# lambdaclass/simpleworks

Measured on AMD Instinct MI355X. Metric: Marlin prove() constraints/sec at 2^20 R1CS; G1 MSM points/sec, higher is better.
Workload: dtype u32 limbs (384-bit Montgomery Fq for G1, 256-bit Fr); 1 GPU; marlin_prove: synthetic R1CS, 2^20 constraints = variables = non-zeros per matrix (|H| = |K| = 2^20), SRS + proving key device resident; per_gpu_units=1048576, multi_gpu=replicas (one proof per rank)

## Files before the change

### simpleworks_amd/_lib.py

```python
import ctypes
import json
import os

import numpy as np

_HERE = os.path.dirname(os.path.abspath(__file__))
LIB_PATH = os.environ.get("SWM_LIB_PATH") or os.path.join(_HERE, "libswmarlin.so")

_u64p = ctypes.POINTER(ctypes.c_uint64)
_u32p = ctypes.POINTER(ctypes.c_uint32)
_vp = ctypes.c_void_p
_sz = ctypes.c_size_t
_int = ctypes.c_int

ABI = {
    "swm_version": (_int, []),
    "swm_strerror": (ctypes.c_char_p, [_int]),
    "swm_init": (_int, [_int, ctypes.POINTER(_vp)]),
    "swm_destroy": (None, [_vp]),
    "swm_last_error": (ctypes.c_char_p, [_vp]),
    "swm_set_stream": (_int, [_vp, _vp]),
    "swm_set_msm_sharding": (_int, [_vp, ctypes.c_uint, ctypes.c_uint, _vp, _vp]),
    "swm_rccl_unique_id": (_int, [ctypes.c_void_p]),
    "swm_rccl_init": (_int, [_vp, ctypes.c_void_p, ctypes.c_uint, ctypes.c_uint]),
# ... 466 lines not shown

    def selftest_ntt_cosets(self, coeffs_mont, log_n, ks):
        src = np.ascontiguousarray(coeffs_mont, dtype=np.uint64).reshape(-1, 4).copy()
        kk = np.ascontiguousarray(ks, dtype=np.uint64).reshape(-1)
        out = np.zeros((kk.size << log_n, 4), dtype=np.uint64)
        self._check(self.lib.swm_selftest_poly(self.h, 9, src.ctypes.data, src.shape[0], log_n, _p64(np.zeros(4, np.uint64)),
                                               _p64(kk), kk.size, out.ctypes.data), "swm_selftest_poly")
        return out.reshape(kk.size, 1 << log_n, 4)

    def selftest_intt_cosets3(self, evals_mont, log_n):
        ev = np.ascontiguousarray(evals_mont, dtype=np.uint64).reshape(-1, 4).copy()
        out = np.zeros_like(ev)
        self._poly(10, ev, ev.shape[0], log_n, None, None, out)
        return out

    def selftest_scan(self, words):
        w = np.ascontiguousarray(words, dtype=np.uint32).reshape(-1)
        out = np.zeros(w.size + 1, dtype=np.uint32)
        self._poly(8, w, w.size, 0, None, None, out)
        return out[:-1], int(out[-1])

    def selftest_sample_fr(self, rng, need):
        out = np.zeros((max(need, 1), 4), dtype=np.uint64)
        self._check(self.lib.swm_selftest_sample_fr(self.h, rng.h, need, _p64(out)), "swm_selftest_sample_fr")
        return out[:need]

    def selftest_mul_throughput(self, which, threads, iters):
        ms = ctypes.c_float(0)
        self._check(self.lib.swm_selftest_mul_throughput(self.h, which, threads, iters, ctypes.byref(ms)),
                    "swm_selftest_mul_throughput")
# ... 2 lines not shown
```

### simpleworks_amd/csrc/devops.cuh

```cuda
#pragma once
#include <chrono>
#include <exception>
#include <functional>
#include <utility>
#include <atomic>
#include "context.h"
#include "ff.cuh"
#include "fill.cuh"
#include "fr29.cuh"
#include "host/chacha.h"
#include "host/marlin_types.h"

namespace swm {

int ntt_run(swm_ctx* ctx, void* d_data, unsigned log_n, int inverse, int coset);
int ntt_run_from(swm_ctx* ctx, void* d_data, unsigned log_n, int inverse, int coset, const void* first_src, size_t src_len);
int ntt_cosets_fwd(swm_ctx* ctx, const void* coeffs, size_t len, unsigned log_n, const unsigned* ks, unsigned ncos, void* out);
int ntt_cosets_inv(swm_ctx* ctx, void* data, unsigned log_n, unsigned ncos);
int ntt_sharded_run(swm_ctx* ctx, void* d_local, unsigned log_n, int inverse, int blocks_in);
struct SpmvPlanHost {
    uint64_t nnz = 0, max_row = 0;
    std::vector<uint32_t> chunks, lrows;
};
struct SpmvPlan {
    uint64_t nnz = 0, max_row = 0;
    const uint32_t* d_chunks = nullptr;
    const uint32_t* d_lrows = nullptr;
    uint32_t n_chunks = 0, n_lrows = 0;
};
void spmv_plan_build(const uint32_t* rowptr, size_t rows, SpmvPlanHost* plan);
int spmv_run(swm_ctx* ctx, const void* d_rowptr, const void* d_col, const void* d_val, const void* d_z, void* d_out,
             size_t rows, const SpmvPlan* plan = nullptr);
int batch_inverse_run(swm_ctx* ctx, void* d, size_t n);
// ... 847 lines not shown
```

### simpleworks_amd/csrc/marlin.hip

```cpp
#include <stdlib.h>
#include <string.h>
#include <algorithm>
#include <chrono>
#include <functional>
#include <memory>
#include "devops.cuh"
#include "g1.cuh"
#include "host/ahp.h"

#include "msm.h"
using namespace swm;

#define LAUNCHX(ctx, name, kernel, grid, block, shmem, ...)                         \
    do {                                                                            \
        prof_begin(ctx, name);                                                      \
        hipLaunchKernelGGL(kernel, grid, block, shmem, (ctx)->stream, __VA_ARGS__); \
        prof_end(ctx);                                                              \
        hip_check(ctx, hipGetLastError(), name);                                    \
    } while (0)

#include "host/pk_codec.h"
#include "host/host_handles.h"
struct swm_srs {
    ~swm_srs() {
// ... 972 lines not shown
}
#ifndef SWM_OUTER_COSETS
#define SWM_OUTER_COSETS 1
#endif
static constexpr uint64_t OUTER_COSETS_MIN_H = 16;
struct Cosets3 {
    Fr p0, p1, p2;
};
__device__ __forceinline__ Cosets3 cosets3_solve(const Fr& u0, const Fr& u1, const Fr& u2, const Fr& iota, const Fr& half) {
    const Fr p1 = fp_mul(fp_sub(u0, u2), half);
    const Fr e = fp_mul(fp_add(u0, u2), half);
    const Fr d = fp_sub(u1, fp_mul(iota, p1));
    return {fp_mul(fp_add(e, d), half), p1, fp_mul(fp_sub(e, d), half)};
}
static Fr fr_half() { return fp_inv(fp_from_u64<Fr>(2)); }
struct RAlphaNumerators {
    Fr n0, n1, n2, n3;
};
RAlphaNumerators r_alpha_numerators(const Fr& alpha, unsigned logH, uint64_t M) {
    Fr aH = alpha;
    for (unsigned i = 0; i < logH; i++) aH = fp_sqr(aH);
    Fr i4 = HDomain(M).gen;
    for (unsigned i = 0; i < logH; i++) i4 = fp_sqr(i4);
    return {fp_sub(aH, fp_one<Fr>()), fp_sub(aH, i4), fp_sub(aH, fp_sqr(i4)), fp_sub(aH, fp_mul(fp_sqr(i4), i4))};
}
struct IndexOnB {
    const Fr *ar, *ac, *arc, *av;
    const Fr *br, *bc, *brc, *bv;
    const Fr *cr, *cc, *crc, *cv;
};
// ... 388 lines not shown
        hip_check(ctx, hipMemcpyAsync(s.e_ra.p + H, e12.p, 2 * H * sizeof(Fr), hipMemcpyDeviceToDevice, ctx->stream), "copy");
    }
    {
        DVec e_t = on_cosets12(ctx, s, s.t_poly.p, H);
        Fr* out = s.q1.p + H;
        const Fr *pra = s.e_ra.p + H, *pza = s.e_za.p, *pzb = s.e_zb.p, *pt = e_t.p, *pz = s.e_z.p;
        ew(ctx, "round2_pointwise", 2 * H, [=] __device__(size_t i) {
            Fr a = pza[i], b = pzb[i];
            Fr summed = fp_add(fp_add(fp_mul(eta_c, fp_mul(a, b)), fp_mul(eta_a, a)), fp_mul(eta_b, b));
            out[i] = fp_sub(fp_mul(pra[i], summed), fp_mul(pz[i], pt[i]));
        });
        s.e_za.release();
        s.e_zb.release();
        s.e_z.release();
    }
    rc_check(ctx, ntt_cosets_inv(ctx, s.q1.p, pk.logH, 3));
    s.h1 = DVec(ctx, 3 * H);
    s.g1x = DVec(ctx, H);
    const Fr* q = s.q1.p;
    const Fr* mp = s.mask.p;
    Fr *h = s.h1.p, *g = s.g1x.p;
    const Fr iota = HDomain(4).gen, half = fr_half();
    ew(ctx, "q1_cosets_solve_div_vh", H, [=] __device__(size_t j) {
        const Cosets3 c = cosets3_solve(q[j], q[j + H], q[j + 2 * H], iota, half);
        const Fr p0 = fp_add(c.p0, mp[j]), p1 = fp_add(c.p1, mp[j + H]), p2 = fp_add(c.p2, mp[j + 2 * H]);
        const Fr hj = fp_add(p1, p2);
        h[j] = hj;
        h[j + H] = p2;
        h[j + 2 * H] = fp_zero<Fr>();
        g[j] = fp_add(p0, hj);
    });
// ... 69 lines not shown
                        {&s.P_t.rand, &s.P_g1.rand, &s.P_h1.rand}, s.comms2.data());
    if (unsat && !ctx->emulated_exchange)
        throw MarlinError(SWM_ERR_UNSATISFIED, "outer sumcheck does not hold: constraint system is not satisfied");
}

void round3_polys(swm_ctx* ctx, const swm_pk& pk, ProveState& s) {
    const uint64_t K = s.K, Bsz = s.Bsz;
    const Fr alpha = s.st.alpha, beta = s.st.beta;
    const Fr eta_a = s.st.eta_a, eta_b = s.st.eta_b, eta_c = s.st.eta_c;
    const Fr vhab = fp_mul(s.dh.vanishing(alpha), s.dh.vanishing(beta));
    s.f = DVec(ctx, K);
    const bool f_cosets = SWM_OUTER_COSETS && !s.sp.r3 && Bsz == 4 * K && K >= OUTER_COSETS_MIN_H;
    DVec f_K;
    {
        DVec inv(ctx, 3 * K);
        for (int m = 0; m < 3; m++) {
            Fr* out = inv.p + (size_t)m * K;
            const Fr *rk = pk.ar[m].row_K.p, *ck = pk.ar[m].col_K.p;
            ew(ctx, "round3_den_K", K, [=] __device__(size_t i) { out[i] = fp_mul(fp_sub(beta, rk[i]), fp_sub(alpha, ck[i])); });
        }
        rc_check(ctx, batch_inverse_run(ctx, inv.p, 3 * K));
        Fr* out = s.f.p;
        const Fr *ia = inv.p, *ib = inv.p + K, *ic = inv.p + 2 * K;
        const Fr *va = pk.ar[0].val_K.p, *vb = pk.ar[1].val_K.p, *vc = pk.ar[2].val_K.p;
        if (f_cosets) {
            f_K = DVec(ctx, K);
            out = f_K.p;
        }
        ew(ctx, "round3_f_K", K, [=] __device__(size_t i) {
            Fr t = fp_add(fp_add(fp_mul(fp_mul(eta_a, va[i]), ia[i]), fp_mul(fp_mul(eta_b, vb[i]), ib[i])),
                          fp_mul(fp_mul(eta_c, vc[i]), ic[i]));
            out[i] = fp_mul(vhab, t);
        });
        if (f_cosets) rc_check(ctx, ntt_run_from(ctx, s.f.p, pk.logK, 1, 0, f_K.p, K));
        else dv_ntt(ctx, s.f, pk.logK, true);
// ... 7 lines not shown
    const Round3Challenges ch{alpha, beta, fp_mul(beta, alpha), eta_a, eta_b, eta_c, vhab};
    if (s.sp.r3) {
        const size_t Bloc = Bsz / s.sp.SG, Bblk = Bloc / s.sp.SG, Kl = K / s.sp.SG, s_rank = s.sp.rank;
        DVec e_f = shard_evals(ctx, s.sp, s.f.p, K, pk.logB);
        DVec ab(ctx, Bloc);
        Fr* out = ab.p;
        const Fr* pf = e_f.p;
        ew(ctx, "round3_pointwise_B", Bloc, [=] __device__(size_t p) {
            const size_t i = Bloc * (p / Bblk) + s_rank * Bblk + (p % Bblk);
            out[p] = round3_a_minus_bf(ix, ch, i, pf[p]);
        });
        rc_check(ctx, ntt_sharded_run(ctx, ab.p, pk.logB, 1, 1));
        DVec loc(ctx, 3 * Kl);
        div_vk(ctx, ab.p, Kl, Bloc, loc.p);
        shard_gather_cyclic(ctx, loc.p, 3 * Kl, s.sp.slog_g, s.h2.p, 3 * K);
    } else if (f_cosets) {
        static const unsigned ks[3] = {1, 2, 3};
        DVec e_f(ctx, 3 * K);
        rc_check(ctx, ntt_cosets_fwd(ctx, s.f.p, K, pk.logK, ks, 3, e_f.p));
        DVec ab(ctx, Bsz);
        Fr* out = ab.p;
        const Fr *pf = e_f.p, *fk = f_K.p;
        const unsigned logK = pk.logK;
        ew(ctx, "round3_pointwise_B", Bsz, [=] __device__(size_t i) {
            const size_t k = i & 3, j = i >> 2;
            out[i] = round3_a_minus_bf(ix, ch, i, k ? pf[((k - 1) << logK) + j] : fk[j]);
        });
        dv_ntt(ctx, ab, pk.logB, true);
        div_vk(ctx, ab.p, K, Bsz, s.h2.p);
    } else {
// ... 826 lines not shown
        return;
    }
    DVec a(ctx, n);
    if (n) a.upload((const Fr*)data, n);
    if (op == 9) {
        unsigned ks[4];
        for (size_t c = 0; c < npieces; c++) ks[c] = (unsigned)pieces[c];
        DVec t(ctx, npieces << m);
        rc_check(ctx, ntt_cosets_fwd(ctx, a.p, n, (unsigned)m, ks, (unsigned)npieces, t.p));
        std::vector<Fr> h = t.download(0, t.n);
        memcpy(out, h.data(), t.n * sizeof(Fr));
        return;
    }
    if (op == 10) {
        const size_t N = (size_t)1 << m;
        rc_check(ctx, ntt_cosets_inv(ctx, a.p, (unsigned)m, 3));
        DVec t(ctx, 3 * N);
        const Fr* u = a.p;
        Fr* o = t.p;
        const Fr iota = HDomain(4).gen, half = fr_half();
        ew(ctx, "cosets3_solve", N, [=] __device__(size_t j) {
            const Cosets3 c = cosets3_solve(u[j], u[j + N], u[j + 2 * N], iota, half);
            o[j] = c.p0;
            o[j + N] = c.p1;
            o[j + 2 * N] = c.p2;
        });
        std::vector<Fr> h = t.download(0, t.n);
        memcpy(out, h.data(), t.n * sizeof(Fr));
        return;
    }
    if (op == 0) {
        suffix_recurrence(ctx, a.p, n, m, zz);
        std::vector<Fr> h = a.download(0, n);
        if (n) memcpy(data, h.data(), n * sizeof(Fr));
    } else if (op == 1) {
        DivResult r = div_linear(ctx, a.p, n, zz);
        std::vector<Fr> h = r.work.download(0, n);
        if (n) memcpy(out, h.data(), n * sizeof(Fr));
    } else if (op == 2) {
        const Fr v = poly_eval(ctx, a.p, n, zz);
        memcpy(out, v.v, sizeof(Fr));
// ... 5 lines not shown
        for (size_t i = 0; i < npieces; i++) items.push_back({a.p + pieces[2 * i], (size_t)pieces[2 * i + 1], res.p + i});
        EvalPoint ep = eval_point(ctx, zz);
        poly_eval_many(ctx, items, ep);
        std::vector<Fr> h = res.download(0, npieces);
        if (npieces) memcpy(out, h.data(), npieces * sizeof(Fr));
    } else {
        DVec t = dv_ntt_from(ctx, a.p, n, (unsigned)m, ((op - 4) & 1) != 0, ((op - 4) & 2) != 0);
        std::vector<Fr> h = t.download(0, t.n);
        memcpy(out, h.data(), t.n * sizeof(Fr));
        std::vector<Fr> s = a.download(0, n);
        if (n) memcpy(data, s.data(), n * sizeof(Fr));
    }
}
int swm_selftest_poly(swm_ctx* ctx, int op, void* data, size_t n, size_t m, const uint64_t z[4], const uint64_t* pieces,
                      size_t npieces, void* out) {
    if (!ctx || op < 0 || op > 10 || (n && !data)) return SWM_ERR_INVALID_ARG;
    if ((op >= 1 && op <= 3 && !z) || (op == 0 && (!z || m == 0)) || (op != 0 && !out) || (op == 3 && npieces && !pieces))
        return SWM_ERR_INVALID_ARG;
    if (op >= 4 && op <= 7 && (m < 1 || m > 28 || n > ((size_t)1 << m))) return SWM_ERR_INVALID_ARG;
    if (op == 9) {
        if (m < 1 || m > 26 || n > ((size_t)2 << m) || npieces < 1 || npieces > 4 || !pieces) return SWM_ERR_INVALID_ARG;
        for (size_t c = 0; c < npieces; c++)
            if (pieces[c] > 3) return SWM_ERR_INVALID_ARG;
    }
    if (op == 10 && (m < 1 || m > 26 || n != ((size_t)3 << m))) return SWM_ERR_INVALID_ARG;
    SWM_ON_DEVICE(ctx);
    SWM_GUARD(ctx, selftest_poly_impl(ctx, op, data, n, m, z, pieces, npieces, out));
}
static void selftest_sample_impl(swm_ctx* ctx, ChaChaRng& rng, size_t need, uint64_t* out_mont) {
    DVec d(ctx, need);
    sample_fr_bulk(ctx, rng, d.p, need);
    std::vector<Fr> h = d.download(0, need);
    if (need) memcpy(out_mont, h.data(), need * sizeof(Fr));
}
int swm_selftest_sample_fr(swm_ctx* ctx, swm_rng* rng, size_t need, uint64_t* out_mont) {
    if (!ctx || !rng || (need && !out_mont)) return SWM_ERR_INVALID_ARG;
    SWM_ON_DEVICE(ctx);
    SWM_GUARD(ctx, selftest_sample_impl(ctx, rng->r, need, out_mont));
}

// ... 70 lines not shown
```

### simpleworks_amd/csrc/ntt.hip

```cpp
#include <atomic>
#include "context.h"
#include "ff.cuh"
#include "fr29.cuh"
#include <string.h>
#include <algorithm>
#include <vector>

namespace swm {

static constexpr int NTT_THREADS = 256;
static constexpr unsigned NTT_MAX_LOG_R = 10;

struct NttPassArgs {
    const Fr* src;
    Fr* dst;
    unsigned log_n, log_r, log_ns;
    const Fr* tw_small;
    const Fr* tw_lo;
    const Fr* tw_hi;
    const Fr* cs_lo;
    const Fr* cs_hi;
    uint64_t src_len;
    const Fr* pass_tw;
    int coset_in;
    int scale_out;
    int coset_out;
    Fr n_inv;
    uint64_t src_cstride, dst_cstride;
    uint32_t cos_k[4];
    int fold_in;
    Fr fold[4];
};

__device__ __forceinline__ Fr two_level_pow(const Fr* lo, const Fr* hi, uint64_t e) {
    Fr a = lo[e & 1023];
    uint64_t h = e >> 10;
    if (h) a = fp_mul(a, hi[h]);
    return a;
}

__device__ __forceinline__ unsigned bitrev_u(unsigned x, unsigned bits) { return bits ? (__brev(x) >> (32 - bits)) : 0u; }

template <int J>
__global__ void __launch_bounds__(NTT_THREADS) ntt_pass(NttPassArgs a) {
    SWM_LIGHT_KERNEL();
    extern __shared__ __align__(16) unsigned char smem_raw[];
    Fr* tile = reinterpret_cast<Fr*>(smem_raw);
    const unsigned R = 1u << a.log_r;
    const uint64_t n = 1ull << a.log_n;
    const uint64_t stride = n >> a.log_r;
    const uint64_t j0 = (uint64_t)blockIdx.x * J;
    const uint64_t ns_mask = (1ull << a.log_ns) - 1;
    const unsigned tw_shift = a.log_n - a.log_ns - a.log_r;
    const Fr* src = a.src + blockIdx.y * a.src_cstride;
    Fr* dst = a.dst + blockIdx.y * a.dst_cstride;
    const uint64_t cs_k = a.cos_k[blockIdx.y];
    for (unsigned e0 = 0; e0 < R * J; e0 += 4 * NTT_THREADS) {
        Fr xs[4];
#pragma unroll
        for (int u = 0; u < 4; u++) {
            unsigned e = e0 + threadIdx.x + u * NTT_THREADS;
            if (e < R * J) {
                const uint64_t at = j0 + e % J + (uint64_t)(e / J) * stride;
                xs[u] = at < a.src_len ? src[at] : fp_zero<Fr>();
                if (a.fold_in && at + n < a.src_len) xs[u] = fp_add(xs[u], fp_mul(a.fold[blockIdx.y], src[at + n]));
            }
        }
#pragma unroll
        for (int u = 0; u < 4; u++) {
            unsigned e = e0 + threadIdx.x + u * NTT_THREADS;
            if (e >= R * J) break;
            unsigned jj = e % J, t = e / J;
            uint64_t idx = j0 + jj + (uint64_t)t * stride;
            Fr x = xs[u];
            if (a.coset_in) x = fp_mul(x, two_level_pow(a.cs_lo, a.cs_hi, idx * cs_k));
            if (a.log_ns != 0 && t != 0) {
                uint64_t k = (j0 + jj) & ns_mask;
                if (k) x = fp_mul(x, two_level_pow(a.tw_lo, a.tw_hi, (k * t) << tw_shift));
            }
            tile[t * J + jj] = x;
// ... 38 lines not shown
        __syncthreads();
    }
    for (unsigned e = threadIdx.x; e < R * J; e += NTT_THREADS) {
        unsigned jj, u;
        if (a.log_ns == 0) {
            u = e % R;
            jj = e / R;
        } else {
            jj = e % J;
            u = e / J;
        }
        uint64_t j = j0 + jj;
        uint64_t k = j & ns_mask;
        uint64_t o = ((j - k) << a.log_r) + k + ((uint64_t)u << a.log_ns);
        Fr x = tile[bitrev_u(u, a.log_r) * J + jj];
        if (a.scale_out) {
            Fr s = a.n_inv;
            if (a.coset_out) s = fp_mul(s, two_level_pow(a.cs_lo, a.cs_hi, o * cs_k));
            x = fp_mul(x, s);
        }
        dst[o] = x;
    }
}

struct LazyPlan {
    Spread29 r2;
    Spread29 s1[6];
    Spread29 s2[6];
    Spread29 s4;
    uint32_t reduce;
    uint32_t out_below_2r;
};
struct NttLazyArgs {
    NttPassArgs a;
    LazyPlan plan;
    int last_pass;
// ... 5 lines not shown
    return a;
}
__device__ __forceinline__ unsigned tile_slot(unsigned idx) { return (idx + (idx >> 5)) * 9; }
__device__ __forceinline__ void tile_put(uint32_t* tile, unsigned idx, const Fr29& x) {
    const unsigned o = tile_slot(idx);
#pragma unroll
    for (int i = 0; i < 9; i++) tile[o + i] = x.l[i];
}
__device__ __forceinline__ Fr29 tile_get(const uint32_t* tile, unsigned idx) {
    const unsigned o = tile_slot(idx);
    Fr29 x;
#pragma unroll
    for (int i = 0; i < 9; i++) x.l[i] = tile[o + i];
    return x;
}
template <int J>
__global__ void __launch_bounds__(NTT_THREADS, 4) ntt_pass_lazy(NttLazyArgs args) {
    SWM_LIGHT_KERNEL();
    extern __shared__ __align__(16) unsigned char smem_raw[];
    uint32_t* tile = reinterpret_cast<uint32_t*>(smem_raw);
    const NttPassArgs& a = args.a;
    const LazyPlan& P = args.plan;
    const unsigned R = 1u << a.log_r;
    const uint64_t n = 1ull << a.log_n;
    const uint64_t stride = n >> a.log_r;
    const uint64_t j0 = (uint64_t)blockIdx.x * J;
    const uint64_t ns_mask = (1ull << a.log_ns) - 1;
    const unsigned tw_shift = a.log_n - a.log_ns - a.log_r;
    const Fr* src = a.src + blockIdx.y * a.src_cstride;
    Fr* dst = a.dst + blockIdx.y * a.dst_cstride;
    const uint64_t cs_k = a.cos_k[blockIdx.y];
    for (unsigned e0 = 0; e0 < R * J; e0 += 4 * NTT_THREADS) {
        Fr xs[4];
#pragma unroll
        for (int u = 0; u < 4; u++) {
            unsigned e = e0 + threadIdx.x + u * NTT_THREADS;
            if (e < R * J) {
                const uint64_t at = j0 + e % J + (uint64_t)(e / J) * stride;
                xs[u] = at < a.src_len ? src[at] : fp_zero<Fr>();
                if (a.fold_in && at + n < a.src_len) xs[u] = fp_add(xs[u], fp_mul(a.fold[blockIdx.y], src[at + n]));
            }
        }
#pragma unroll
        for (int u = 0; u < 4; u++) {
            unsigned e = e0 + threadIdx.x + u * NTT_THREADS;
            if (e >= R * J) break;
            unsigned jj = e % J, t = e / J;
            uint64_t idx = j0 + jj + (uint64_t)t * stride;
            Fr29 x = fr29_unpack(xs[u]);
            if (a.coset_in) x = fr29_mul_fenced(x, two_level_pow29(a.cs_lo, a.cs_hi, idx * cs_k));
            if (a.log_ns != 0) {
                uint64_t k = (j0 + jj) & ns_mask;
                const Fr29 tw = a.pass_tw ? fr29_unpack(a.pass_tw[((uint64_t)t << a.log_ns) + k])
                                          : two_level_pow29(a.tw_lo, a.tw_hi, (k * t) << tw_shift);
                x = fr29_mul_fenced(x, tw);
// ... 46 lines not shown
        __syncthreads();
    }
    for (unsigned e = threadIdx.x; e < R * J; e += NTT_THREADS) {
        unsigned jj, u;
        if (a.log_ns == 0) {
            u = e % R;
            jj = e / R;
        } else {
            jj = e % J;
            u = e / J;
        }
        uint64_t j = j0 + jj;
        uint64_t k = j & ns_mask;
        uint64_t o = ((j - k) << a.log_r) + k + ((uint64_t)u << a.log_ns);
        Fr29 x = tile_get(tile, bitrev_u(u, a.log_r) * J + jj);
        if (a.scale_out) {
            Fr29 sc = fr29_unpack(a.n_inv);
            if (a.coset_out) sc = fr29_mul_fenced(two_level_pow29(a.cs_lo, a.cs_hi, o * cs_k), sc);
            x = fr29_canonical(fr29_mul_fenced(x, sc), true);
        } else if (args.last_pass) {
            x = fr29_canonical(x, P.out_below_2r != 0);
        }
        dst[o] = fr29_pack(x);
    }
}

static Fr host_root_of_unity(unsigned log_n, bool inverse) {
    Fr w;
    const uint32_t root[8] = SWM_FR_ROOT47_MONT;
    for (int i = 0; i < 8; i++) w.v[i] = root[i];
    for (unsigned i = log_n; i < 47; i++) w = fp_sqr(w);
    if (inverse) w = fp_inv(w);
    return w;
}

static int upload_powers(swm_ctx* ctx, const Fr& base, size_t count, void** out, bool lazy29 = false) {
    std::vector<Fr> h(count);
    Fr cur = lazy29 ? fp_from_u64<Fr>(32) : fp_one<Fr>();
// ... 124 lines not shown
        P.s1[st] = lazy_spread(2 * B, 1);
        P.s2[st] = lazy_spread(4 * B, 2);
        const bool red = 4 * B > 64 || st + 1 == nsteps;
        if (red) P.reduce |= 1u << st;
        B = red ? 4 : 4 * B;
    }
    P.s4 = lazy_spread(4, 1);
    P.out_below_2r = B <= 2 ? 1u : 0u;
    return P;
}

int ntt_run_from(swm_ctx* ctx, void* d_data, unsigned log_n, int inverse, int coset, const void* first_src, size_t src_len);
int ntt_run(swm_ctx* ctx, void* d_data, unsigned log_n, int inverse, int coset) {
    return ntt_run_from(ctx, d_data, log_n, inverse, coset, nullptr, 0);
}
static int ntt_run_multi(swm_ctx* ctx, void* d_data, unsigned log_n, int inverse, int coset, const void* first_src, size_t src_len,
                         unsigned ncos, const unsigned* ks);
int ntt_run_from(swm_ctx* ctx, void* d_data, unsigned log_n, int inverse, int coset, const void* first_src, size_t src_len) {
    if (first_src && src_len > (1ull << std::min(log_n, 62u))) src_len = 1ull << log_n;
    return ntt_run_multi(ctx, d_data, log_n, inverse, coset ? 1 : 0, first_src, src_len, 1, nullptr);
}
int ntt_cosets_fwd(swm_ctx* ctx, const void* coeffs, size_t len, unsigned log_n, const unsigned* ks, unsigned ncos, void* out) {
    if (ncos < 1 || ncos > 4 || log_n > 28 || len > (2ull << log_n)) return set_err(ctx, SWM_ERR_INVALID_ARG, "ntt cosets: bad shape");
    for (unsigned c = 0; c < ncos; c++)
        if (ks[c] > 3) return set_err(ctx, SWM_ERR_INVALID_ARG, "ntt cosets: coset index > 3");
    return ntt_run_multi(ctx, out, log_n, 0, 2, coeffs, len, ncos, ks);
}
int ntt_cosets_inv(swm_ctx* ctx, void* data, unsigned log_n, unsigned ncos) {
    if (ncos < 1 || ncos > 4 || log_n > 28) return set_err(ctx, SWM_ERR_INVALID_ARG, "ntt cosets: bad shape");
    const unsigned ks[4] = {0, 1, 2, 3};
    return ntt_run_multi(ctx, data, log_n, 1, 2, nullptr, 0, ncos, ks);
}
static int ntt_run_multi(swm_ctx* ctx, void* d_data, unsigned log_n, int inverse, int coset, const void* first_src, size_t src_len,
                         unsigned ncos, const unsigned* ks) {
    if (log_n > 30) return set_err(ctx, SWM_ERR_INVALID_ARG, "ntt: log_n > 30 unsupported");
    const uint64_t n = 1ull << log_n;
    for (unsigned c = 0; c < ncos; c++) {
        ctx->stat_ntt_calls++;
        ctx->log_call('n', log_n);
        ctx->stat_ntt_elems += n;
    }
    Fr* data = reinterpret_cast<Fr*>(d_data);
    const uint64_t total = n * ncos;
    const unsigned maxr = NTT_MAX_LOG_R;
    static const bool lazy = sw(SW_NTT_LAZY) != 0;
    NttTables *rt = nullptr, *ct = nullptr;
    SWM_TRY(get_root_tables_form(ctx, log_n, inverse, lazy, &rt));
    if (coset == 1) SWM_TRY(get_coset_tables(ctx, log_n, inverse, &ct, lazy));
    if (coset == 2) SWM_TRY(get_root_tables_form(ctx, log_n + 2, inverse, lazy, &ct));
// ... 8 lines not shown
    if (lazy) n_inv = fp_mul(n_inv, fp_from_u64<Fr>(32));
    unsigned npass = log_n <= maxr ? 1 : (log_n + maxr - 1) / maxr;
    unsigned radices[8];
    {
        unsigned rem = log_n;
        for (unsigned p = 0; p < npass; p++) {
            unsigned r = (rem + (npass - p) - 1) / (npass - p);
            radices[p] = r;
            rem -= r;
        }
    }
    Fr *tmp = nullptr, *tmp2 = nullptr;
    SWM_TRY(scratch(ctx, "ntt.tmp", total * sizeof(Fr), (void**)&tmp));
    if (npass % 2 == 1 && npass >= 3) SWM_TRY(scratch(ctx, "ntt.tmp2", total * sizeof(Fr), (void**)&tmp2));
    const Fr* src = first_src ? reinterpret_cast<const Fr*>(first_src) : data;
    if (npass == 1 && !first_src) {
        SWM_HIP(ctx, hipMemcpyAsync(tmp, data, total * sizeof(Fr), hipMemcpyDeviceToDevice, ctx->stream));
        src = tmp;
    }
    unsigned log_ns = 0;
    for (unsigned p = 0; p < npass; p++) {
        NttPassArgs a;
        a.src = src;
        if (p == npass - 1) a.dst = data;
        else if (tmp2) a.dst = (p % 2 == 0) ? tmp : tmp2;
        else a.dst = (src == tmp) ? data : tmp;
        a.src_len = (p == 0 && first_src) ? (uint64_t)src_len : n;
        a.log_n = log_n;
        a.log_r = radices[p];
        a.log_ns = log_ns;
        SWM_TRY(get_small_table(ctx, a.log_r, inverse, &a.tw_small, lazy));
        a.tw_lo = reinterpret_cast<const Fr*>(rt->lo);
        a.tw_hi = reinterpret_cast<const Fr*>(rt->hi);
        a.cs_lo = ct ? reinterpret_cast<const Fr*>(ct->lo) : nullptr;
        a.cs_hi = ct ? reinterpret_cast<const Fr*>(ct->hi) : nullptr;
        a.pass_tw = nullptr;
        if (lazy && log_ns != 0) SWM_TRY(get_pass_table(ctx, log_n, inverse, log_ns, a.log_r, rt, &a.pass_tw));
        a.coset_in = (coset && !inverse && p == 0) ? 1 : 0;
        a.scale_out = (inverse && p == npass - 1) ? 1 : 0;
        a.coset_out = (coset && inverse && p == npass - 1) ? 1 : 0;
        a.n_inv = n_inv;
        a.src_cstride = (p == 0 && first_src) ? 0 : n;
        a.dst_cstride = n;
        a.fold_in = (coset == 2 && a.coset_in && src_len > n) ? 1 : 0;
        for (unsigned c = 0; c < 4; c++) {
            a.cos_k[c] = coset == 2 ? (c < ncos ? ks[c] : 0) : 1;
            a.fold[c] = fold[c];
        }
        uint64_t cols = n >> a.log_r;
        if (lazy) {
            NttLazyArgs la;
            la.a = a;
            la.plan = lazy_plan(a.log_r, (p > 0 || a.coset_in) ? 2u : 1u);
            la.last_pass = p == npass - 1 ? 1 : 0;
            unsigned J = 1;
            if (npass > 1) {
                J = (log_n >= 19 ? 1024u : 512u) >> a.log_r;
                if (J < 1) J = 1;
                if (J > 16) J = 16;
                while (J > cols) J >>= 1;
            }
            const size_t elems = (size_t)J << a.log_r;
            size_t shmem = (elems + (elems >> 5) + 1) * 36;
            if (shmem < 64) shmem = 64;
            dim3 grid((unsigned)(cols / J), ncos), block(NTT_THREADS);
            if (shmem > 64 * 1024) {
                static std::atomic<size_t> granted[64];
                if (J != 1 || shmem > 160 * 1024) return set_err(ctx, SWM_ERR_INVALID_ARG, "ntt: tile does not fit LDS");
                if (granted[ctx->device & 63].load() < shmem) {
                    SWM_HIP(ctx, hipFuncSetAttribute((const void*)ntt_pass_lazy<1>, hipFuncAttributeMaxDynamicSharedMemorySize, (int)shmem));
                    granted[ctx->device & 63].store(shmem);
                }
            }
            switch (J) {
                case 1: SWM_LAUNCH(ctx, "ntt_pass", ntt_pass_lazy<1>, grid, block, shmem, la); break;
                case 2: SWM_LAUNCH(ctx, "ntt_pass", ntt_pass_lazy<2>, grid, block, shmem, la); break;
                case 4: SWM_LAUNCH(ctx, "ntt_pass", ntt_pass_lazy<4>, grid, block, shmem, la); break;
                case 8: SWM_LAUNCH(ctx, "ntt_pass", ntt_pass_lazy<8>, grid, block, shmem, la); break;
                default: SWM_LAUNCH(ctx, "ntt_pass", ntt_pass_lazy<16>, grid, block, shmem, la); break;
            }
        } else if (npass == 1) {
            size_t shmem = sizeof(Fr) << a.log_r;
            if (shmem < 64) shmem = 64;
            SWM_LAUNCH(ctx, "ntt_pass", ntt_pass<1>, dim3((unsigned)cols, ncos), dim3(NTT_THREADS), shmem, a);
        } else {
            unsigned J = (log_n >= 19 ? 1024u : 512u) >> a.log_r;
            if (J < 1) J = 1;
            if (J > 16) J = 16;
            while (J > cols) J >>= 1;
            size_t shmem = (sizeof(Fr) * J) << a.log_r;
            dim3 grid((unsigned)(cols / J), ncos), block(NTT_THREADS);
            switch (J) {
                case 1: SWM_LAUNCH(ctx, "ntt_pass", ntt_pass<1>, grid, block, shmem, a); break;
                case 2: SWM_LAUNCH(ctx, "ntt_pass", ntt_pass<2>, grid, block, shmem, a); break;
                case 4: SWM_LAUNCH(ctx, "ntt_pass", ntt_pass<4>, grid, block, shmem, a); break;
                case 8: SWM_LAUNCH(ctx, "ntt_pass", ntt_pass<8>, grid, block, shmem, a); break;
                default: SWM_LAUNCH(ctx, "ntt_pass", ntt_pass<16>, grid, block, shmem, a); break;
            }
        }
        log_ns += a.log_r;
        src = a.dst;
    }
    return SWM_OK;
}


__global__ void __launch_bounds__(256) ntt_shard_twiddle(Fr* __restrict__ v, size_t count, const Fr* __restrict__ lo,
// ... 71 lines not shown
```

Baseline: 22.98 million constraints/s.

## Fuse three-coset solve and vanishing division into final inverse NTT pass in round 3

Adds a solve3 variant of the final inverse-NTT pass that processes all three cosets in one block, applies the coset shift, and combines the three results through a precomputed 3x3 interpolation matrix. The matrix also folds in n^-1 and the inverse vanishing polynomial per coset. Round 3's h2 computation uses this path, replacing separate unscaled inverse NTTs, solve kernels and vanishing-division passes. The three per-matrix denominator kernels are also merged into one launch. The fused last pass runs one grid over cosets serially instead of a coset grid dimension, which lowers parallelism in that pass and adds read-back traffic for the third coset.

```diff
diff --git a/simpleworks_amd/_lib.py b/simpleworks_amd/_lib.py
--- a/simpleworks_amd/_lib.py
+++ b/simpleworks_amd/_lib.py
@@ -504,6 +504,15 @@
         self._poly(10, ev, ev.shape[0], log_n, None, None, out)
         return out
 
+    def selftest_intt_cosets_solve3(self, evals_mont, log_n, ks, times_vanishing=False):
+        ev = np.ascontiguousarray(evals_mont, dtype=np.uint64).reshape(-1, 4).copy()
+        kk = np.ascontiguousarray(ks, dtype=np.uint64).reshape(3)
+        flag = np.array([1 if times_vanishing else 0, 0, 0, 0], dtype=np.uint64)
+        out = np.zeros_like(ev)
+        self._check(self.lib.swm_selftest_poly(self.h, 11, ev.ctypes.data, ev.shape[0], log_n, _p64(flag), _p64(kk), 3,
+                                               out.ctypes.data), "swm_selftest_poly")
+        return out
+
     def selftest_scan(self, words):
         w = np.ascontiguousarray(words, dtype=np.uint32).reshape(-1)
         out = np.zeros(w.size + 1, dtype=np.uint32)
diff --git a/simpleworks_amd/csrc/devops.cuh b/simpleworks_amd/csrc/devops.cuh
--- a/simpleworks_amd/csrc/devops.cuh
+++ b/simpleworks_amd/csrc/devops.cuh
@@ -16,7 +16,8 @@
 int ntt_run(swm_ctx* ctx, void* d_data, unsigned log_n, int inverse, int coset);
 int ntt_run_from(swm_ctx* ctx, void* d_data, unsigned log_n, int inverse, int coset, const void* first_src, size_t src_len);
 int ntt_cosets_fwd(swm_ctx* ctx, const void* coeffs, size_t len, unsigned log_n, const unsigned* ks, unsigned ncos, void* out);
-int ntt_cosets_inv(swm_ctx* ctx, void* data, unsigned log_n, unsigned ncos);
+int ntt_cosets_inv(swm_ctx* ctx, void* data, unsigned log_n, const unsigned* ks, unsigned ncos);
+int ntt_cosets_inv_solve3(swm_ctx* ctx, const void* evals, unsigned log_n, const unsigned* ks, const void* scale, void* out);
 int ntt_sharded_run(swm_ctx* ctx, void* d_local, unsigned log_n, int inverse, int blocks_in);
 struct SpmvPlanHost {
     uint64_t nnz = 0, max_row = 0;
diff --git a/simpleworks_amd/csrc/marlin.hip b/simpleworks_amd/csrc/marlin.hip
--- a/simpleworks_amd/csrc/marlin.hip
+++ b/simpleworks_amd/csrc/marlin.hip
@@ -1010,6 +1010,17 @@
     return {fp_mul(fp_add(e, d), half), p1, fp_mul(fp_sub(e, d), half)};
 }
 static Fr fr_half() { return fp_inv(fp_from_u64<Fr>(2)); }
+#ifndef SWM_ROUND3_COSETS
+#define SWM_ROUND3_COSETS 1
+#endif
+static void inv_vanishing_on_cosets(const unsigned* ks, Fr out[3]) {
+    const Fr w4 = HDomain(4).gen;
+    for (int c = 0; c < 3; c++) {
+        Fr x = fp_one<Fr>();
+        for (unsigned e = 0; e < ks[c]; e++) x = fp_mul(x, w4);
+        out[c] = fp_inv(fp_sub(x, fp_one<Fr>()));
+    }
+}
 struct RAlphaNumerators {
     Fr n0, n1, n2, n3;
 };
@@ -1428,7 +1439,8 @@
         s.e_zb.release();
         s.e_z.release();
     }
-    rc_check(ctx, ntt_cosets_inv(ctx, s.q1.p, pk.logH, 3));
+    static const unsigned ks012[3] = {0, 1, 2};
+    rc_check(ctx, ntt_cosets_inv(ctx, s.q1.p, pk.logH, ks012, 3));
     s.h1 = DVec(ctx, 3 * H);
     s.g1x = DVec(ctx, H);
     const Fr* q = s.q1.p;
@@ -1528,11 +1540,24 @@
     DVec f_K;
     {
         DVec inv(ctx, 3 * K);
+#if SWM_ROUND3_COSETS
+        {
+            Fr* out = inv.p;
+            const Fr *r0 = pk.ar[0].row_K.p, *r1 = pk.ar[1].row_K.p, *r2 = pk.ar[2].row_K.p;
+            const Fr *c0 = pk.ar[0].col_K.p, *c1 = pk.ar[1].col_K.p, *c2 = pk.ar[2].col_K.p;
+            ew(ctx, "round3_den_K", 3 * K, [=] __device__(size_t p) {
+                const size_t m = p / K, i = p - m * K;
+                const Fr *rk = m == 0 ? r0 : m == 1 ? r1 : r2, *ck = m == 0 ? c0 : m == 1 ? c1 : c2;
+                out[p] = fp_mul(fp_sub(beta, rk[i]), fp_sub(alpha, ck[i]));
+            });
+        }
+#else
         for (int m = 0; m < 3; m++) {
             Fr* out = inv.p + (size_t)m * K;
             const Fr *rk = pk.ar[m].row_K.p, *ck = pk.ar[m].col_K.p;
             ew(ctx, "round3_den_K", K, [=] __device__(size_t i) { out[i] = fp_mul(fp_sub(beta, rk[i]), fp_sub(alpha, ck[i])); });
         }
+#endif
         rc_check(ctx, batch_inverse_run(ctx, inv.p, 3 * K));
         Fr* out = s.f.p;
         const Fr *ia = inv.p, *ib = inv.p + K, *ic = inv.p + 2 * K;
@@ -1570,6 +1595,20 @@
         DVec loc(ctx, 3 * Kl);
         div_vk(ctx, ab.p, Kl, Bloc, loc.p);
         shard_gather_cyclic(ctx, loc.p, 3 * Kl, s.sp.slog_g, s.h2.p, 3 * K);
+    } else if (f_cosets && SWM_ROUND3_COSETS) {
+        static const unsigned ks[3] = {1, 2, 3};
+        DVec e_f(ctx, 3 * K);
+        rc_check(ctx, ntt_cosets_fwd(ctx, s.f.p, K, pk.logK, ks, 3, e_f.p));
+        DVec ab(ctx, 3 * K);
+        Fr* out = ab.p;
+        const Fr* pf = e_f.p;
+        ew(ctx, "round3_pointwise_B", 3 * K, [=] __device__(size_t p) {
+            const size_t j = p / 3, c = p - 3 * j, at = c * K + j;
+            out[at] = round3_a_minus_bf(ix, ch, 4 * j + c + 1, pf[at]);
+        });
+        Fr vk_inv[3];
+        inv_vanishing_on_cosets(ks, vk_inv);
+        rc_check(ctx, ntt_cosets_inv_solve3(ctx, ab.p, pk.logK, ks, vk_inv, s.h2.p));
     } else if (f_cosets) {
         static const unsigned ks[3] = {1, 2, 3};
         DVec e_f(ctx, 3 * K);
@@ -2426,7 +2465,8 @@
     }
     if (op == 10) {
         const size_t N = (size_t)1 << m;
-        rc_check(ctx, ntt_cosets_inv(ctx, a.p, (unsigned)m, 3));
+        static const unsigned ks012[3] = {0, 1, 2};
+        rc_check(ctx, ntt_cosets_inv(ctx, a.p, (unsigned)m, ks012, 3));
         DVec t(ctx, 3 * N);
         const Fr* u = a.p;
         Fr* o = t.p;
@@ -2437,6 +2477,17 @@
             o[j + N] = c.p1;
             o[j + 2 * N] = c.p2;
         });
+        std::vector<Fr> h = t.download(0, t.n);
+        memcpy(out, h.data(), t.n * sizeof(Fr));
+        return;
+    }
+    if (op == 11) {
+        unsigned ks[3];
+        for (int c = 0; c < 3; c++) ks[c] = (unsigned)pieces[c];
+        Fr scale[3];
+        if (z && z[0]) inv_vanishing_on_cosets(ks, scale);
+        DVec t(ctx, n);
+        rc_check(ctx, ntt_cosets_inv_solve3(ctx, a.p, (unsigned)m, ks, z && z[0] ? scale : nullptr, t.p));
         std::vector<Fr> h = t.download(0, t.n);
         memcpy(out, h.data(), t.n * sizeof(Fr));
         return;
@@ -2472,7 +2523,7 @@
 }
 int swm_selftest_poly(swm_ctx* ctx, int op, void* data, size_t n, size_t m, const uint64_t z[4], const uint64_t* pieces,
                       size_t npieces, void* out) {
-    if (!ctx || op < 0 || op > 10 || (n && !data)) return SWM_ERR_INVALID_ARG;
+    if (!ctx || op < 0 || op > 11 || (n && !data)) return SWM_ERR_INVALID_ARG;
     if ((op >= 1 && op <= 3 && !z) || (op == 0 && (!z || m == 0)) || (op != 0 && !out) || (op == 3 && npieces && !pieces))
         return SWM_ERR_INVALID_ARG;
     if (op >= 4 && op <= 7 && (m < 1 || m > 28 || n > ((size_t)1 << m))) return SWM_ERR_INVALID_ARG;
@@ -2482,6 +2533,11 @@
             if (pieces[c] > 3) return SWM_ERR_INVALID_ARG;
     }
     if (op == 10 && (m < 1 || m > 26 || n != ((size_t)3 << m))) return SWM_ERR_INVALID_ARG;
+    if (op == 11) {
+        if (m < 1 || m > 26 || n != ((size_t)3 << m) || npieces != 3 || !pieces) return SWM_ERR_INVALID_ARG;
+        for (size_t c = 0; c < 3; c++)
+            if (pieces[c] > 3 || (z && z[0] && pieces[c] == 0)) return SWM_ERR_INVALID_ARG;
+    }
     SWM_ON_DEVICE(ctx);
     SWM_GUARD(ctx, selftest_poly_impl(ctx, op, data, n, m, z, pieces, npieces, out));
 }
diff --git a/simpleworks_amd/csrc/ntt.hip b/simpleworks_amd/csrc/ntt.hip
--- a/simpleworks_amd/csrc/ntt.hip
+++ b/simpleworks_amd/csrc/ntt.hip
@@ -30,6 +30,7 @@
     uint32_t cos_k[4];
     int fold_in;
     Fr fold[4];
+    Fr sol[9];
 };
 
 __device__ __forceinline__ Fr two_level_pow(const Fr* lo, const Fr* hi, uint64_t e) {
@@ -41,20 +42,29 @@
 
 __device__ __forceinline__ unsigned bitrev_u(unsigned x, unsigned bits) { return bits ? (__brev(x) >> (32 - bits)) : 0u; }
 
-template <int J>
-__global__ void __launch_bounds__(NTT_THREADS) ntt_pass(NttPassArgs a) {
-    SWM_LIGHT_KERNEL();
-    extern __shared__ __align__(16) unsigned char smem_raw[];
-    Fr* tile = reinterpret_cast<Fr*>(smem_raw);
+__device__ __forceinline__ void solve3_store(const NttPassArgs& a, Fr* out, uint64_t n, uint64_t o, unsigned c, const Fr& x) {
+    if (c < 2) {
+        out[c * n + o] = x;
+        return;
+    }
+    const Fr x0 = out[o], x1 = out[n + o];
+#pragma unroll
+    for (int m = 0; m < 3; m++)
+        out[m * n + o] = fp_add(fp_add(fp_mul(a.sol[3 * m], x0), fp_mul(a.sol[3 * m + 1], x1)), fp_mul(a.sol[3 * m + 2], x));
+}
+
+template <int J, bool SOLVE3>
+__device__ __forceinline__ void ntt_pass_tile(const NttPassArgs& a, Fr* tile, const unsigned c) {
     const unsigned R = 1u << a.log_r;
     const uint64_t n = 1ull << a.log_n;
     const uint64_t stride = n >> a.log_r;
     const uint64_t j0 = (uint64_t)blockIdx.x * J;
     const uint64_t ns_mask = (1ull << a.log_ns) - 1;
     const unsigned tw_shift = a.log_n - a.log_ns - a.log_r;
-    const Fr* src = a.src + blockIdx.y * a.src_cstride;
-    Fr* dst = a.dst + blockIdx.y * a.dst_cstride;
-    const uint64_t cs_k = a.cos_k[blockIdx.y];
+    const Fr* src = a.src + c * a.src_cstride;
+    Fr* dst = a.dst + c * a.dst_cstride;
+    (void)dst;
+    const uint64_t cs_k = a.cos_k[c];
     for (unsigned e0 = 0; e0 < R * J; e0 += 4 * NTT_THREADS) {
         Fr xs[4];
 #pragma unroll
@@ -63,7 +73,7 @@
             if (e < R * J) {
                 const uint64_t at = j0 + e % J + (uint64_t)(e / J) * stride;
                 xs[u] = at < a.src_len ? src[at] : fp_zero<Fr>();
-                if (a.fold_in && at + n < a.src_len) xs[u] = fp_add(xs[u], fp_mul(a.fold[blockIdx.y], src[at + n]));
+                if (a.fold_in && at + n < a.src_len) xs[u] = fp_add(xs[u], fp_mul(a.fold[c], src[at + n]));
             }
         }
 #pragma unroll
@@ -132,12 +142,33 @@
         uint64_t k = j & ns_mask;
         uint64_t o = ((j - k) << a.log_r) + k + ((uint64_t)u << a.log_ns);
         Fr x = tile[bitrev_u(u, a.log_r) * J + jj];
-        if (a.scale_out) {
-            Fr s = a.n_inv;
-            if (a.coset_out) s = fp_mul(s, two_level_pow(a.cs_lo, a.cs_hi, o * cs_k));
-            x = fp_mul(x, s);
-        }
-        dst[o] = x;
+        if constexpr (SOLVE3) {
+            if (cs_k) x = fp_mul(x, two_level_pow(a.cs_lo, a.cs_hi, o * cs_k));
+            solve3_store(a, a.dst, n, o, c, x);
+        } else {
+            if (a.scale_out) {
+                Fr s = a.n_inv;
+                if (a.coset_out) s = fp_mul(s, two_level_pow(a.cs_lo, a.cs_hi, o * cs_k));
+                x = fp_mul(x, s);
+            }
+            dst[o] = x;
+        }
+    }
+}
+template <int J>
+__global__ void __launch_bounds__(NTT_THREADS) ntt_pass(NttPassArgs a) {
+    SWM_LIGHT_KERNEL();
+    extern __shared__ __align__(16) unsigned char smem_raw[];
+    ntt_pass_tile<J, false>(a, reinterpret_cast<Fr*>(smem_raw), blockIdx.y);
+}
+template <int J>
+__global__ void __launch_bounds__(NTT_THREADS) ntt_pass_solve3(NttPassArgs a) {
+    SWM_LIGHT_KERNEL();
+    extern __shared__ __align__(16) unsigned char smem_raw[];
+#pragma unroll 1
+    for (unsigned c = 0; c < 3; c++) {
+        if (c) __syncthreads();
+        ntt_pass_tile<J, true>(a, reinterpret_cast<Fr*>(smem_raw), c);
     }
 }
 
@@ -173,11 +204,8 @@
     for (int i = 0; i < 9; i++) x.l[i] = tile[o + i];
     return x;
 }
-template <int J>
-__global__ void __launch_bounds__(NTT_THREADS, 4) ntt_pass_lazy(NttLazyArgs args) {
-    SWM_LIGHT_KERNEL();
-    extern __shared__ __align__(16) unsigned char smem_raw[];
-    uint32_t* tile = reinterpret_cast<uint32_t*>(smem_raw);
+template <int J, bool SOLVE3>
+__device__ __forceinline__ void ntt_pass_lazy_tile(const NttLazyArgs& args, uint32_t* tile, const unsigned c) {
     const NttPassArgs& a = args.a;
     const LazyPlan& P = args.plan;
     const unsigned R = 1u << a.log_r;
@@ -186,9 +214,9 @@
     const uint64_t j0 = (uint64_t)blockIdx.x * J;
     const uint64_t ns_mask = (1ull << a.log_ns) - 1;
     const unsigned tw_shift = a.log_n - a.log_ns - a.log_r;
-    const Fr* src = a.src + blockIdx.y * a.src_cstride;
-    Fr* dst = a.dst + blockIdx.y * a.dst_cstride;
-    const uint64_t cs_k = a.cos_k[blockIdx.y];
+    const Fr* src = a.src + c * a.src_cstride;
+    Fr* dst = a.dst + c * a.dst_cstride;
+    const uint64_t cs_k = a.cos_k[c];
     for (unsigned e0 = 0; e0 < R * J; e0 += 4 * NTT_THREADS) {
         Fr xs[4];
 #pragma unroll
@@ -197,7 +225,7 @@
             if (e < R * J) {
                 const uint64_t at = j0 + e % J + (uint64_t)(e / J) * stride;
                 xs[u] = at < a.src_len ? src[at] : fp_zero<Fr>();
-                if (a.fold_in && at + n < a.src_len) xs[u] = fp_add(xs[u], fp_mul(a.fold[blockIdx.y], src[at + n]));
+                if (a.fold_in && at + n < a.src_len) xs[u] = fp_add(xs[u], fp_mul(a.fold[c], src[at + n]));
             }
         }
 #pragma unroll
@@ -274,6 +302,11 @@
         uint64_t k = j & ns_mask;
         uint64_t o = ((j - k) << a.log_r) + k + ((uint64_t)u << a.log_ns);
         Fr29 x = tile_get(tile, bitrev_u(u, a.log_r) * J + jj);
+        if constexpr (SOLVE3) {
+            x = fr29_canonical(fr29_mul_fenced(x, two_level_pow29(a.cs_lo, a.cs_hi, o * cs_k)), true);
+            solve3_store(a, a.dst, n, o, c, fr29_pack(x));
+            continue;
+        }
         if (a.scale_out) {
             Fr29 sc = fr29_unpack(a.n_inv);
             if (a.coset_out) sc = fr29_mul_fenced(two_level_pow29(a.cs_lo, a.cs_hi, o * cs_k), sc);
@@ -282,6 +315,22 @@
             x = fr29_canonical(x, P.out_below_2r != 0);
         }
         dst[o] = fr29_pack(x);
+    }
+}
+template <int J>
+__global__ void __launch_bounds__(NTT_THREADS, 4) ntt_pass_lazy(NttLazyArgs args) {
+    SWM_LIGHT_KERNEL();
+    extern __shared__ __align__(16) unsigned char smem_raw[];
+    ntt_pass_lazy_tile<J, false>(args, reinterpret_cast<uint32_t*>(smem_raw), blockIdx.y);
+}
+template <int J>
+__global__ void __launch_bounds__(NTT_THREADS, 4) ntt_pass_lazy_solve3(NttLazyArgs args) {
+    SWM_LIGHT_KERNEL();
+    extern __shared__ __align__(16) unsigned char smem_raw[];
+#pragma unroll 1
+    for (unsigned c = 0; c < 3; c++) {
+        if (c) __syncthreads();
+        ntt_pass_lazy_tile<J, true>(args, reinterpret_cast<uint32_t*>(smem_raw), c);
     }
 }
 
@@ -436,8 +485,12 @@
 int ntt_run(swm_ctx* ctx, void* d_data, unsigned log_n, int inverse, int coset) {
     return ntt_run_from(ctx, d_data, log_n, inverse, coset, nullptr, 0);
 }
+struct Solve3 {
+    Fr m[9];
+    Fr* out;
+};
 static int ntt_run_multi(swm_ctx* ctx, void* d_data, unsigned log_n, int inverse, int coset, const void* first_src, size_t src_len,
-                         unsigned ncos, const unsigned* ks);
+                         unsigned ncos, const unsigned* ks, const Solve3* solve = nullptr);
 int ntt_run_from(swm_ctx* ctx, void* d_data, unsigned log_n, int inverse, int coset, const void* first_src, size_t src_len) {
     if (first_src && src_len > (1ull << std::min(log_n, 62u))) src_len = 1ull << log_n;
     return ntt_run_multi(ctx, d_data, log_n, inverse, coset ? 1 : 0, first_src, src_len, 1, nullptr);
@@ -448,13 +501,37 @@
         if (ks[c] > 3) return set_err(ctx, SWM_ERR_INVALID_ARG, "ntt cosets: coset index > 3");
     return ntt_run_multi(ctx, out, log_n, 0, 2, coeffs, len, ncos, ks);
 }
-int ntt_cosets_inv(swm_ctx* ctx, void* data, unsigned log_n, unsigned ncos) {
+int ntt_cosets_inv(swm_ctx* ctx, void* data, unsigned log_n, const unsigned* ks, unsigned ncos) {
     if (ncos < 1 || ncos > 4 || log_n > 28) return set_err(ctx, SWM_ERR_INVALID_ARG, "ntt cosets: bad shape");
-    const unsigned ks[4] = {0, 1, 2, 3};
+    for (unsigned c = 0; c < ncos; c++)
+        if (ks[c] > 3) return set_err(ctx, SWM_ERR_INVALID_ARG, "ntt cosets: coset index > 3");
     return ntt_run_multi(ctx, data, log_n, 1, 2, nullptr, 0, ncos, ks);
 }
+int ntt_cosets_inv_solve3(swm_ctx* ctx, const void* evals, unsigned log_n, const unsigned* ks, const void* scale, void* out) {
+    if (log_n > 28 || evals == out) return set_err(ctx, SWM_ERR_INVALID_ARG, "ntt cosets: bad shape");
+    const Fr w4 = host_root_of_unity(2, false);
+    Fr x[3];
+    for (unsigned c = 0; c < 3; c++) {
+        if (ks[c] > 3 || (c > 0 && ks[c] == ks[0]) || (c == 2 && ks[2] == ks[1]))
+            return set_err(ctx, SWM_ERR_INVALID_ARG, "ntt cosets: three distinct coset indices <= 3");
+        x[c] = fp_one<Fr>();
+        for (unsigned e = 0; e < ks[c]; e++) x[c] = fp_mul(x[c], w4);
+    }
+    const Fr n_inv = fp_inv(fp_from_u64<Fr>(1ull << log_n));
+    Solve3 sv;
+    sv.out = reinterpret_cast<Fr*>(out);
+    for (unsigned c = 0; c < 3; c++) {
+        const Fr &xa = x[(c + 1) % 3], &xb = x[(c + 2) % 3];
+        Fr f = fp_mul(fp_inv(fp_mul(fp_sub(x[c], xa), fp_sub(x[c], xb))), n_inv);
+        if (scale) f = fp_mul(f, reinterpret_cast<const Fr*>(scale)[c]);
+        sv.m[c] = fp_mul(fp_mul(xa, xb), f);
+        sv.m[3 + c] = fp_sub(fp_zero<Fr>(), fp_mul(fp_add(xa, xb), f));
+        sv.m[6 + c] = f;
+    }
+    return ntt_run_multi(ctx, const_cast<void*>(evals), log_n, 1, 2, nullptr, 0, 3, ks, &sv);
+}
 static int ntt_run_multi(swm_ctx* ctx, void* d_data, unsigned log_n, int inverse, int coset, const void* first_src, size_t src_len,
-                         unsigned ncos, const unsigned* ks) {
+                         unsigned ncos, const unsigned* ks, const Solve3* solve) {
     if (log_n > 30) return set_err(ctx, SWM_ERR_INVALID_ARG, "ntt: log_n > 30 unsupported");
     const uint64_t n = 1ull << log_n;
     for (unsigned c = 0; c < ncos; c++) {
@@ -493,7 +570,7 @@
     SWM_TRY(scratch(ctx, "ntt.tmp", total * sizeof(Fr), (void**)&tmp));
     if (npass % 2 == 1 && npass >= 3) SWM_TRY(scratch(ctx, "ntt.tmp2", total * sizeof(Fr), (void**)&tmp2));
     const Fr* src = first_src ? reinterpret_cast<const Fr*>(first_src) : data;
-    if (npass == 1 && !first_src) {
+    if (npass == 1 && !first_src && !solve) {
         SWM_HIP(ctx, hipMemcpyAsync(tmp, data, total * sizeof(Fr), hipMemcpyDeviceToDevice, ctx->stream));
         src = tmp;
     }
@@ -501,7 +578,9 @@
     for (unsigned p = 0; p < npass; p++) {
         NttPassArgs a;
         a.src = src;
-        if (p == npass - 1) a.dst = data;
+        const bool solve_pass = solve && p == npass - 1;
+        if (solve_pass) a.dst = solve->out;
+        else if (p == npass - 1) a.dst = data;
         else if (tmp2) a.dst = (p % 2 == 0) ? tmp : tmp2;
         else a.dst = (src == tmp) ? data : tmp;
         a.src_len = (p == 0 && first_src) ? (uint64_t)src_len : n;
@@ -526,6 +605,7 @@
             a.cos_k[c] = coset == 2 ? (c < ncos ? ks[c] : 0) : 1;
             a.fold[c] = fold[c];
         }
+        for (unsigned i = 0; i < 9; i++) a.sol[i] = solve ? solve->m[i] : fp_zero<Fr>();
         uint64_t cols = n >> a.log_r;
         if (lazy) {
             NttLazyArgs la;
@@ -542,16 +622,23 @@
             const size_t elems = (size_t)J << a.log_r;
             size_t shmem = (elems + (elems >> 5) + 1) * 36;
             if (shmem < 64) shmem = 64;
-            dim3 grid((unsigned)(cols / J), ncos), block(NTT_THREADS);
+            dim3 grid((unsigned)(cols / J), solve_pass ? 1 : ncos), block(NTT_THREADS);
             if (shmem > 64 * 1024) {
                 static std::atomic<size_t> granted[64];
-                if (J != 1 || shmem > 160 * 1024) return set_err(ctx, SWM_ERR_INVALID_ARG, "ntt: tile does not fit LDS");
+                if (J != 1 || shmem > 160 * 1024 || solve_pass) return set_err(ctx, SWM_ERR_INVALID_ARG, "ntt: tile does not fit LDS");
                 if (granted[ctx->device & 63].load() < shmem) {
                     SWM_HIP(ctx, hipFuncSetAttribute((const void*)ntt_pass_lazy<1>, hipFuncAttributeMaxDynamicSharedMemorySize, (int)shmem));
                     granted[ctx->device & 63].store(shmem);
                 }
             }
-            switch (J) {
+            if (solve_pass) switch (J) {
+                case 1: SWM_LAUNCH(ctx, "ntt_pass", ntt_pass_lazy_solve3<1>, grid, block, shmem, la); break;
+                case 2: SWM_LAUNCH(ctx, "ntt_pass", ntt_pass_lazy_solve3<2>, grid, block, shmem, la); break;
+                case 4: SWM_LAUNCH(ctx, "ntt_pass", ntt_pass_lazy_solve3<4>, grid, block, shmem, la); break;
+                case 8: SWM_LAUNCH(ctx, "ntt_pass", ntt_pass_lazy_solve3<8>, grid, block, shmem, la); break;
+                default: SWM_LAUNCH(ctx, "ntt_pass", ntt_pass_lazy_solve3<16>, grid, block, shmem, la); break;
+            }
+            else switch (J) {
                 case 1: SWM_LAUNCH(ctx, "ntt_pass", ntt_pass_lazy<1>, grid, block, shmem, la); break;
                 case 2: SWM_LAUNCH(ctx, "ntt_pass", ntt_pass_lazy<2>, grid, block, shmem, la); break;
                 case 4: SWM_LAUNCH(ctx, "ntt_pass", ntt_pass_lazy<4>, grid, block, shmem, la); break;
@@ -561,15 +648,23 @@
         } else if (npass == 1) {
             size_t shmem = sizeof(Fr) << a.log_r;
             if (shmem < 64) shmem = 64;
-            SWM_LAUNCH(ctx, "ntt_pass", ntt_pass<1>, dim3((unsigned)cols, ncos), dim3(NTT_THREADS), shmem, a);
+            if (solve_pass) SWM_LAUNCH(ctx, "ntt_pass", ntt_pass_solve3<1>, dim3((unsigned)cols), dim3(NTT_THREADS), shmem, a);
+            else SWM_LAUNCH(ctx, "ntt_pass", ntt_pass<1>, dim3((unsigned)cols, ncos), dim3(NTT_THREADS), shmem, a);
         } else {
             unsigned J = (log_n >= 19 ? 1024u : 512u) >> a.log_r;
             if (J < 1) J = 1;
             if (J > 16) J = 16;
             while (J > cols) J >>= 1;
             size_t shmem = (sizeof(Fr) * J) << a.log_r;
-            dim3 grid((unsigned)(cols / J), ncos), block(NTT_THREADS);
-            switch (J) {
+            dim3 grid((unsigned)(cols / J), solve_pass ? 1 : ncos), block(NTT_THREADS);
+            if (solve_pass) switch (J) {
+                case 1: SWM_LAUNCH(ctx, "ntt_pass", ntt_pass_solve3<1>, grid, block, shmem, a); break;
+                case 2: SWM_LAUNCH(ctx, "ntt_pass", ntt_pass_solve3<2>, grid, block, shmem, a); break;
+                case 4: SWM_LAUNCH(ctx, "ntt_pass", ntt_pass_solve3<4>, grid, block, shmem, a); break;
+                case 8: SWM_LAUNCH(ctx, "ntt_pass", ntt_pass_solve3<8>, grid, block, shmem, a); break;
+                default: SWM_LAUNCH(ctx, "ntt_pass", ntt_pass_solve3<16>, grid, block, shmem, a); break;
+            }
+            else switch (J) {
                 case 1: SWM_LAUNCH(ctx, "ntt_pass", ntt_pass<1>, grid, block, shmem, a); break;
                 case 2: SWM_LAUNCH(ctx, "ntt_pass", ntt_pass<2>, grid, block, shmem, a); break;
                 case 4: SWM_LAUNCH(ctx, "ntt_pass", ntt_pass<4>, grid, block, shmem, a); break;
```

After: 23.11 million constraints/s (median of 6 runs). About the same (+0.6%).
